# scroll-tech/zkevm-circuits

Hardware: NVIDIA H100
Metric: SuperCircuit-shaped k=20 create_proof seconds (halo2 KZG/SHPLONK, Blake2b transcript) (lower is better)
Workload: dtype u256 (8x u32 Montgomery limbs, BN254 Fr/Fq)

## Files before the change

### zkevm-circuits_b200/csrc/expr.cu

```cuda
#include <type_traits>
#include "common.cuh"
#include "expr.cuh"

namespace zkb {

struct ExprLaunch {
    const Instr *code;
    uint32_t ncode;
    const Fr *const *cols;
    const Fr *consts;
    Fr *const *outs;
    uint32_t log_n;
    uint32_t out_stride;
    uint32_t out_offset;
};

template <int NREGS, int THREADS, bool SMEM>
struct RegFile {
    uint4 *lo, *hi;
    Fr loc[SMEM ? 1 : NREGS];
    __device__ __forceinline__ RegFile(uint4 *base) : lo(base + threadIdx.x), hi(base + NREGS * THREADS + threadIdx.x) {}
    __device__ __forceinline__ Fr get(uint32_t r) const {
        if (!SMEM) return loc[r];
        const uint4 a = lo[r * THREADS], b = hi[r * THREADS];
// ... 61 lines not shown
        case OP_MUL_RC + FORM_RK: x = regs.get(in.a); y = cst(in.imm); goto mul;
        case OP_MUL_RC + FORM_KR: x = cst(in.imm); y = regs.get(in.a); goto mul;
        case OP_MUL_RC + FORM_CC: x = col(in.imm); y = col(arg()); goto mul;
        case OP_MUL_RC + FORM_CK: x = col(in.imm); y = cst(arg()); goto mul;
        case OP_MUL_RC + FORM_KC: x = cst(in.imm); y = col(arg()); goto mul;
        case OP_NEG: regs.set(in.dst, fp_neg(regs.get(in.a))); continue;
        case OP_FLAG:
            if constexpr (FLAG) {
                const uint32_t b = __ballot_sync(0xffffffffu, tid < (1u << L.log_n) && !regs.get(in.a).is_zero());
                const uint32_t word = tid >> 5;
                if ((threadIdx.x & 31) == 0 && word < L.words) L.bits[(size_t)in.imm * L.words + word] = b;
            }
            continue;
        case OP_HORNER: case OP_HORNER_C:
            if constexpr (!FLAG) acc = fp_add(fp_mul(acc, cst(in.imm)), in.op == OP_HORNER ? regs.get(in.a) : col(arg()));
            continue;
        case OP_HORNER2: case OP_HORNER2_C:
            if constexpr (!FLAG) acc2 = fp_add(fp_mul(acc2, cst(in.imm)), in.op == OP_HORNER2 ? regs.get(in.a) : col(arg()));
            continue;
        case OP_FOLD: case OP_FOLD_C:
            if constexpr (FLAG) continue;
            else { x = acc; y = cst(in.imm); z = in.op == OP_FOLD ? regs.get(in.a) : col(arg()); w = acc2; goto mac; }
        case OP_HORNER_M: case OP_HORNER2_M:
            if constexpr (FLAG) continue;
            else if constexpr (!SMEM) {
                const Fr t = fp_mul(regs.get(in.a), regs.get(in.b));
                if (in.op == OP_HORNER_M) acc = fp_add(fp_mul(acc, cst(in.imm)), t);
                else acc2 = fp_add(fp_mul(acc2, cst(in.imm)), t);
                continue;
            } else { x = in.op == OP_HORNER_M ? acc : acc2; y = cst(in.imm); z = regs.get(in.a); w = regs.get(in.b); goto mac; }
        case OP_STORE:
            if constexpr (!FLAG) fp_store(L.outs[in.imm] + (size_t)row * L.out_stride + L.out_offset, regs.get(in.a));
            continue;
        case OP_STOREACC:
            if constexpr (!FLAG) fp_store(L.outs[in.imm & 0xffu] + (size_t)row * L.out_stride + L.out_offset, fp_mul(acc, cst(in.imm >> 8)));
            continue;
        case OP_CLEARACC: acc = Fr::zero(); continue;
        default: continue;
        }
    add: regs.set(in.dst, fp_add(x, y)); continue;
    sub: regs.set(in.dst, fp_sub(x, y)); continue;
    mul: regs.set(in.dst, fp_mul(x, y)); continue;
    mac: {
        const Fr r = fp_mul_add_mul(x, y, z, w);
        if (in.op == OP_HORNER2_M) acc2 = r;
        else {
            acc = r;
            if (in.op != OP_HORNER_M) acc2 = Fr::zero();
        }
    }
    }
}

template <int NREGS, int THREADS, bool SMEM>
__global__ void __launch_bounds__(THREADS) expr_kernel(ExprLaunch L) {
    const uint32_t row = blockIdx.x * blockDim.x + threadIdx.x;
    if (row >= (1u << L.log_n)) return;
    run_program<NREGS, THREADS, SMEM>(L, row);
}

template <int NREGS, int THREADS, bool SMEM>
__global__ void __launch_bounds__(THREADS) expr_flag_kernel(FlagLaunch L) {
    run_program<NREGS, THREADS, SMEM>(L, blockIdx.x * blockDim.x + threadIdx.x);
}

template <class Launch, int NREGS, int THREADS, void (*KERNEL)(Launch)>
static int32_t launch_smem(const Launch &L, uint32_t n, cudaStream_t st) {
    constexpr size_t bytes = (size_t)NREGS * THREADS * 32;
    static bool attr_set[64] = {};
    int dev = 0;
    cudaGetDevice(&dev);
    if (bytes > 48 * 1024 && dev < 64 && !attr_set[dev]) {
        ZKB_CUDA(cudaFuncSetAttribute(KERNEL, cudaFuncAttributeMaxDynamicSharedMemorySize, (int)bytes));
        attr_set[dev] = true;
    }
    KERNEL<<<(n + THREADS - 1) / THREADS, THREADS, bytes, st>>>(L);
    return ZKB_OK;
}

int32_t expr_run_device(zkb_ctx *ctx, const Instr *d_code, uint32_t ncode, int nregs, const Fr *const *d_cols, const Fr *d_consts,
                        Fr *const *d_outs, uint32_t log_n, uint32_t out_stride, uint32_t out_offset, cudaStream_t st) {
    ExprLaunch L{d_code, ncode, d_cols, d_consts, d_outs, log_n, out_stride, out_offset};
    const uint32_t n = 1u << log_n;
    const unsigned blocks = (n + 127) / 128;
    ProfScope ps_(ctx, PROF_EXPR, st);
    if (nregs <= 8) ZKB_TRY((launch_smem<ExprLaunch, 8, 128, expr_kernel<8, 128, true>>(L, n, st)));
    else if (nregs <= 16) ZKB_TRY((launch_smem<ExprLaunch, 16, 128, expr_kernel<16, 128, true>>(L, n, st)));
    else expr_kernel<64, 128, false><<<blocks, 128, 0, st>>>(L);
    ctx->launches++;
    ZKB_CUDA(cudaGetLastError());
    return ZKB_OK;
}

int32_t expr_flag_run_device(zkb_ctx *ctx, const Instr *d_code, uint32_t ncode, int nregs, const Fr *const *d_cols, const Fr *d_consts,
                             uint32_t *bits, uint32_t words, uint32_t log_n, cudaStream_t st) {
    FlagLaunch L{d_code, ncode, d_cols, d_consts, bits, words, log_n};
    const uint32_t n = 1u << log_n;
    if (nregs <= 8) ZKB_TRY((launch_smem<FlagLaunch, 8, 128, expr_flag_kernel<8, 128, true>>(L, n, st)));
    else if (nregs <= 16) ZKB_TRY((launch_smem<FlagLaunch, 16, 128, expr_flag_kernel<16, 128, true>>(L, n, st)));
    else expr_flag_kernel<64, 128, false><<<(n + 127) / 128, 128, 0, st>>>(L);
    ctx->launches++;
    ZKB_CUDA(cudaGetLastError());
    return ZKB_OK;
}

}
```

### zkevm-circuits_b200/csrc/expr.cuh

```cuda
#pragma once
#include <stdint.h>
#include <algorithm>
#include <array>
#include <map>
#include <string>
#include <tuple>
#include <vector>
#include "common.cuh"

namespace zkb {

enum : uint8_t {
    OP_LOADCOL = 0,
    OP_LOADCONST = 1,
    OP_ADD = 2,
    OP_SUB = 3,
    OP_MUL = 4,
    OP_NEG = 5,
    OP_HORNER = 6,
    OP_STORE = 7,
    OP_STOREACC = 8,
    OP_CLEARACC = 9,
    OP_HORNER2 = 10,
    OP_FOLD = 11,
    OP_FLAG = 12,
    OP_ARG = 13,
    FORM_RC = 0, FORM_CR = 1, FORM_RK = 2, FORM_KR = 3, FORM_CC = 4, FORM_CK = 5, FORM_KC = 6,
    OP_ADD_RC = 16,
    OP_SUB_RC = 24,
    OP_MUL_RC = 32,
    OP_HORNER_C = 40,
    OP_HORNER2_C = 41,
    OP_FOLD_C = 42,
    OP_HORNER_M = 43,
    OP_HORNER2_M = 44,
};

struct alignas(8) Instr {
    uint8_t op, dst, a, b;
    uint32_t imm;
};

constexpr int EXPR_MAX_REGS = 64;

struct ENode {
    uint8_t kind;
    uint32_t a, b;
};

class ExprBuilder {
public:
    std::vector<ENode> nodes;
    std::vector<Fr> consts;
    std::vector<uint32_t> degree;

    uint32_t col(uint32_t slot, int32_t rot) { return intern(0, slot, (uint32_t)rot); }
    uint32_t constant(const Fr &v) {
        std::array<uint32_t, 8> key;
        for (int i = 0; i < 8; ++i) key[i] = v.l[i];
        auto it = const_index.find(key);
        uint32_t idx;
        if (it == const_index.end()) {
            idx = (uint32_t)consts.size();
            consts.push_back(v);
            const_index.emplace(key, idx);
        } else idx = it->second;
        return intern(1, idx, 0);
    }
    uint32_t add(uint32_t x, uint32_t y) { return intern(2, x, y); }
    uint32_t sub(uint32_t x, uint32_t y) { return intern(3, x, y); }
    uint32_t mul(uint32_t x, uint32_t y) { return intern(4, x, y); }
    uint32_t neg(uint32_t x) { return intern(5, x, 0); }
    uint32_t const_slot(const Fr &v) {
        uint32_t n = constant(v);
        return nodes[n].a;
    }
    void columns(uint32_t root, std::vector<char> &seen, std::vector<char> &used) const {
        std::vector<uint32_t> stack{root};
        while (!stack.empty()) {
            const uint32_t v = stack.back();
            stack.pop_back();
            if (seen[v]) continue;
            seen[v] = 1;
            const ENode &e = nodes[v];
            if (e.kind == 0) used[e.a] = 1;
            else if (e.kind >= 2) {
                stack.push_back(e.a);
                if (e.kind != 5) stack.push_back(e.b);
            }
        }
    }

private:
    std::map<std::tuple<uint8_t, uint32_t, uint32_t>, uint32_t> index;
    std::map<std::array<uint32_t, 8>, uint32_t> const_index;
    uint32_t intern(uint8_t kind, uint32_t a, uint32_t b) {
        auto key = std::make_tuple(kind, a, b);
        auto it = index.find(key);
        if (it != index.end()) return it->second;
        nodes.push_back(ENode{kind, a, b});
        degree.push_back(kind == 0 ? 1 : kind == 1 ? 0 : kind == 4 ? degree[a] + degree[b] : kind == 5 ? degree[a] : std::max(degree[a], degree[b]));
        index.emplace(key, (uint32_t)nodes.size() - 1);
        return (uint32_t)nodes.size() - 1;
    }
};

class ProgramBuilder {
public:
    explicit ProgramBuilder(ExprBuilder &eb) : eb(eb) {}
    std::vector<Instr> code;
    int max_regs_used = 0;
    std::string error;

    enum RootAction { HORNER, STORE, HORNER2, FOLD, FLAG };
    struct Root { uint32_t node; RootAction action; uint32_t imm; };
    bool scope(const std::vector<Root> &roots);
    void clear_acc() { code.push_back(Instr{OP_CLEARACC, 0, 0, 0, 0}); }
    void store_acc(uint32_t out_slot, uint32_t scale_const_index) {
        code.push_back(Instr{OP_STOREACC, 0, 0, 0, out_slot | (scale_const_index << 8)});
    }

private:
    ExprBuilder &eb;
    void fuse(size_t begin);
    static void merge_products(std::vector<Instr> &code);
};

inline void ProgramBuilder::fuse(size_t begin) {
    auto is_arith = [](uint8_t op) { return op == OP_ADD || op == OP_SUB || op == OP_MUL; };
    auto is_root = [](uint8_t op) { return op == OP_HORNER || op == OP_HORNER2 || op == OP_FOLD; };
    auto is_load = [](uint8_t op) { return op == OP_LOADCOL || op == OP_LOADCONST; };
    auto reads = [&](const Instr &in, int s) {
        if (is_arith(in.op)) return true;
        return s == 0 && (in.op == OP_NEG || is_root(in.op) || in.op == OP_STORE || in.op == OP_FLAG);
    };
    auto writes = [&](const Instr &in) { return is_load(in.op) || is_arith(in.op) || in.op == OP_NEG; };
    const size_t end = code.size();
    std::vector<std::array<int64_t, 2>> src(end - begin, {-1, -1});
    for (size_t i = begin; i < end; ++i) {
        if (!is_load(code[i].op)) continue;
        const uint8_t r = code[i].dst;
        int uses = 0, slot = -1;
        size_t user = 0;
        for (size_t j = i + 1; j < end && uses < 2; ++j) {
            for (int s = 0; s < 2; ++s)
                if (reads(code[j], s) && (s == 0 ? code[j].a : code[j].b) == r) { ++uses; user = j; slot = s; }
            if (writes(code[j]) && code[j].dst == r) break;
        }
        if (uses != 1) continue;
        const uint8_t op = code[user].op;
        if (is_arith(op) || (is_root(op) && code[i].op == OP_LOADCOL)) src[user - begin][slot] = (int64_t)i;
    }
    auto kind = [&](const std::array<int64_t, 2> &s, int k) { return s[k] < 0 ? 'R' : code[s[k]].op == OP_LOADCOL ? 'C' : 'K'; };
    std::vector<bool> fused(end - begin, false);
    for (auto &s : src) {
        if (kind(s, 0) == 'K' && kind(s, 1) == 'K') s[1] = -1;
        for (int k = 0; k < 2; ++k)
            if (s[k] >= 0) fused[s[k] - begin] = true;
    }
    std::vector<Instr> out;
    for (size_t i = begin; i < end; ++i) {
        const Instr in = code[i];
        const auto &s = src[i - begin];
        if (fused[i - begin]) continue;
        if (s[0] < 0 && s[1] < 0) { out.push_back(in); continue; }
        if (is_root(in.op)) {
            const uint8_t op = in.op == OP_HORNER ? OP_HORNER_C : in.op == OP_HORNER2 ? OP_HORNER2_C : OP_FOLD_C;
            out.push_back(Instr{op, 0, 0, 0, in.imm});
            out.push_back(Instr{OP_ARG, 0, 0, 0, code[s[0]].imm});
            continue;
        }
        const char ka = kind(s, 0), kb = kind(s, 1);
        const int form = ka == 'R' ? (kb == 'C' ? FORM_RC : FORM_RK)
                       : kb == 'R' ? (ka == 'C' ? FORM_CR : FORM_KR)
                       : ka == 'C' ? (kb == 'C' ? FORM_CC : FORM_CK) : FORM_KC;
        const uint8_t base = in.op == OP_ADD ? OP_ADD_RC : in.op == OP_SUB ? OP_SUB_RC : OP_MUL_RC;
        const int first = s[0] >= 0 ? 0 : 1;
        const uint8_t reg = ka == 'R' ? in.a : in.b;
        out.push_back(Instr{(uint8_t)(base + form), in.dst, (uint8_t)(form < FORM_CC ? reg : 0), 0, code[s[first]].imm});
// ... 4 lines not shown
    code.insert(code.end(), out.begin(), out.end());
}

inline void ProgramBuilder::merge_products(std::vector<Instr> &code) {
    const size_t n = code.size();
    auto reg_reads = [](const Instr &in, int s) {
        const uint8_t op = in.op;
        if (op == OP_ADD || op == OP_SUB || op == OP_MUL) return true;
        if (s != 0) return false;
        if (op == OP_NEG || op == OP_HORNER || op == OP_HORNER2 || op == OP_FOLD || op == OP_STORE || op == OP_FLAG) return true;
        return op >= OP_ADD_RC && op < OP_MUL_RC + 8 && (op & 7) < FORM_CC;
    };
    auto reg_writes = [](const Instr &in) {
        const uint8_t op = in.op;
        return op == OP_LOADCOL || op == OP_LOADCONST || op == OP_ADD || op == OP_SUB || op == OP_MUL || op == OP_NEG ||
               (op >= OP_ADD_RC && op < OP_MUL_RC + 8);
    };
    std::vector<int64_t> reader(n, -1);
    for (size_t i = 0; i < n; ++i) {
        const Instr &m = code[i];
        if (m.op != OP_MUL) continue;
        int uses = 0;
        size_t user = 0;
        for (size_t j = i + 1; j < n && uses < 2; ++j) {
            for (int s = 0; s < 2; ++s)
                if (reg_reads(code[j], s) && (s == 0 ? code[j].a : code[j].b) == m.dst) { ++uses; user = j; }
            if (reg_writes(code[j]) && code[j].dst == m.dst) break;
        }
        if (uses != 1) continue;
        bool intact = true;
        for (size_t j = i + 1; j < user; ++j)
            if (reg_writes(code[j]) && (code[j].dst == m.a || code[j].dst == m.b)) intact = false;
        if (intact) reader[i] = (int64_t)user;
    }
    std::vector<int64_t> prod(n, -1);
    for (size_t i = 0; i < n; ++i)
        if (reader[i] >= 0 && (code[reader[i]].op == OP_HORNER || code[reader[i]].op == OP_HORNER2)) prod[reader[i]] = (int64_t)i;
    std::vector<bool> merged(n, false);
    std::vector<Instr> out;
    for (size_t j = 0; j < n; ++j) {
        Instr in = code[j];
        if (prod[j] >= 0) {
            in = Instr{(uint8_t)(in.op == OP_HORNER ? OP_HORNER_M : OP_HORNER2_M), 0, code[prod[j]].a, code[prod[j]].b, in.imm};
            merged[prod[j]] = true;
        }
        out.push_back(in);
    }
    code.clear();
    for (size_t j = 0; j < n; ++j)
        if (!merged[j]) code.push_back(out[j]);
}

inline bool ProgramBuilder::scope(const std::vector<Root> &roots) {
    const size_t begin = code.size();
    std::map<uint32_t, int> refs;
    std::vector<uint32_t> stack;
    std::map<uint32_t, bool> seen;
    for (auto &r : roots) {
        refs[r.node]++;
        if (!seen[r.node]) { seen[r.node] = true; stack.push_back(r.node); }
    }
    while (!stack.empty()) {
        uint32_t n = stack.back();
        stack.pop_back();
        const ENode &e = eb.nodes[n];
        if (e.kind >= 2) {
            uint32_t ch[2] = {e.a, e.b};
            int nch = e.kind == 5 ? 1 : 2;
            for (int i = 0; i < nch; ++i) {
                refs[ch[i]]++;
                if (!seen[ch[i]]) { seen[ch[i]] = true; stack.push_back(ch[i]); }
            }
        }
    }
    std::map<uint32_t, int> reg_of;
    std::vector<int> free_regs;
    for (int i = EXPR_MAX_REGS - 1; i >= 0; --i) free_regs.push_back(i);
    auto alloc = [&]() -> int {
        if (free_regs.empty()) return -1;
        int r = free_regs.back();
        free_regs.pop_back();
        if (r + 1 > max_regs_used) max_regs_used = r + 1;
        return r;
    };
    auto release_use = [&](uint32_t n) {
        if (--refs[n] == 0) {
            free_regs.push_back(reg_of[n]);
            reg_of.erase(n);
        }
    };
    struct Frame { uint32_t node; int state; };
    for (auto &r : roots) {
        if (!reg_of.count(r.node)) {
            std::vector<Frame> st;
            st.push_back({r.node, 0});
            while (!st.empty()) {
                Frame &f = st.back();
                const ENode e = eb.nodes[f.node];
                if (reg_of.count(f.node)) { st.pop_back(); continue; }
                if (e.kind < 2) {
                    int rg = alloc();
                    if (rg < 0) { error = "expression needs more than 64 live registers"; return false; }
                    if (e.kind == 0) code.push_back(Instr{OP_LOADCOL, (uint8_t)rg, 0, 0, (e.a & 0xffffu) | ((uint32_t)(uint16_t)(int16_t)(int32_t)e.b << 16)});
                    else code.push_back(Instr{OP_LOADCONST, (uint8_t)rg, 0, 0, e.a});
                    reg_of[f.node] = rg;
                    st.pop_back();
                    continue;
                }
                const int nch = e.kind == 5 ? 1 : 2;
                if (f.state == 0) {
                    f.state = 1;
                    if (!reg_of.count(e.a)) { st.push_back({e.a, 0}); continue; }
                }
                if (f.state == 1) {
                    f.state = 2;
                    if (nch == 2 && !reg_of.count(e.b)) { st.push_back({e.b, 0}); continue; }
                }
                const int ra = reg_of[e.a];
                const int rb = nch == 2 ? reg_of[e.b] : 0;
                const uint32_t me = f.node;
                release_use(e.a);
                if (nch == 2) release_use(e.b);
                int rg = alloc();
                if (rg < 0) { error = "expression needs more than 64 live registers"; return false; }
                uint8_t op = e.kind == 2 ? OP_ADD : e.kind == 3 ? OP_SUB : e.kind == 4 ? OP_MUL : OP_NEG;
                code.push_back(Instr{op, (uint8_t)rg, (uint8_t)ra, (uint8_t)rb, 0});
                reg_of[me] = rg;
                st.pop_back();
            }
        }
        const int rr = reg_of[r.node];
        if (r.action == HORNER) code.push_back(Instr{OP_HORNER, 0, (uint8_t)rr, 0, r.imm});
        else if (r.action == HORNER2) code.push_back(Instr{OP_HORNER2, 0, (uint8_t)rr, 0, r.imm});
        else if (r.action == FOLD) code.push_back(Instr{OP_FOLD, 0, (uint8_t)rr, 0, r.imm});
        else if (r.action == FLAG) code.push_back(Instr{OP_FLAG, 0, (uint8_t)rr, 0, r.imm});
        else code.push_back(Instr{OP_STORE, 0, (uint8_t)rr, 0, r.imm});
        release_use(r.node);
    }
    fuse(begin);
    return true;
}

int32_t expr_run_device(zkb_ctx *ctx, const Instr *d_code, uint32_t ncode, int nregs, const Fr *const *d_cols, const Fr *d_consts,
                        Fr *const *d_outs, uint32_t log_n, uint32_t out_stride, uint32_t out_offset, cudaStream_t st);
int32_t expr_flag_run_device(zkb_ctx *ctx, const Instr *d_code, uint32_t ncode, int nregs, const Fr *const *d_cols, const Fr *d_consts,
                             uint32_t *bits, uint32_t words, uint32_t log_n, cudaStream_t st);

struct DeviceProgram {
    Instr *code = nullptr;
    uint32_t ncode = 0;
    int nregs = 0;
    Fr *consts = nullptr;
};
inline int32_t upload_program(DevPool &pool, const ProgramBuilder &pb, const ExprBuilder &eb, DeviceProgram &dp, cudaStream_t st) {
    dp.ncode = (uint32_t)pb.code.size();
    dp.nregs = pb.max_regs_used;
    ZKB_TRY(pool.alloc(pb.code.size() * sizeof(Instr) + 8, (void **)&dp.code));
    ZKB_TRY(pool.alloc(eb.consts.size() * sizeof(Fr) + 32, (void **)&dp.consts));
    ZKB_CUDA(cudaMemcpyAsync(dp.code, pb.code.data(), pb.code.size() * sizeof(Instr), cudaMemcpyHostToDevice, st));
    ZKB_CUDA(cudaMemcpyAsync(dp.consts, eb.consts.data(), eb.consts.size() * sizeof(Fr), cudaMemcpyHostToDevice, st));
    ZKB_CUDA(cudaStreamSynchronize(st));
    return ZKB_OK;
}
template <class T>
inline int32_t upload_table(DevPool &pool, const std::vector<T *> &host, T ***dev, cudaStream_t st) {
    ZKB_TRY(pool.alloc(host.size() * sizeof(T *) + 8, (void **)dev));
    ZKB_CUDA(cudaMemcpyAsync(*dev, host.data(), host.size() * sizeof(T *), cudaMemcpyHostToDevice, st));
    ZKB_CUDA(cudaStreamSynchronize(st));
    return ZKB_OK;
// ... 16 lines not shown
```

### zkevm-circuits_b200/csrc/prover.cu

```cuda
#include "common.cuh"
#include "csf.cuh"
#include "expr.cuh"
#include "lookup.cuh"
#include "transcript.cuh"
#include <algorithm>
#include <memory>
#include <string.h>
#include <stdlib.h>
#include <time.h>

namespace zkb {

__global__ void set_one_kernel(Fr *a, uint64_t idx) { fp_store(a + idx, Fr::one()); }
__global__ void fill_range_one_kernel(Fr *a, uint64_t from, uint64_t to) {
    uint64_t i = from + blockIdx.x * (uint64_t)blockDim.x + threadIdx.x;
    if (i < to) fp_store(a + i, Fr::one());
}
__global__ void mul_arrays_kernel(const Fr *__restrict__ a, const Fr *__restrict__ b, Fr *__restrict__ out, uint64_t n) {
    uint64_t i = blockIdx.x * (uint64_t)blockDim.x + threadIdx.x;
    if (i < n) fp_store(out + i, fp_mul(fp_load(a + i), fp_load(b + i)));
}
__global__ void scale_const_kernel(Fr *__restrict__ a, Fr c, uint64_t n) {
    uint64_t i = blockIdx.x * (uint64_t)blockDim.x + threadIdx.x;
    if (i < n) fp_store(a + i, fp_mul(fp_load(a + i), c));
// ... 784 lines not shown
        const uint32_t g = group_of(eb.degree[sel] + d);
        const int64_t s = next, r = (int64_t)rests.size();
        for (uint32_t v : rests)
            if (!emit(g, {{v, ProgramBuilder::HORNER2, eb.const_slot(y)}})) return false;
        const uint32_t fold = eb.const_slot(fp_pow_u64(y, (uint64_t)(last[g] < 0 ? r : s - last[g] - 1 + r)));
        if (!emit(g, {{sel, ProgramBuilder::FOLD, fold}})) return false;
        reads[g].push_back(sel);
        reads[g].insert(reads[g].end(), rests.begin(), rests.end());
        last[g] = s + r - 1;
        next += r;
        count[g] += (uint32_t)r;
        return true;
    }
    Fr tail(uint32_t g) const { return fp_pow_u64(y, (uint64_t)(next - 1 - last[g])); }
};

static int32_t quotient_gates(const Csf &cs, const std::vector<Fr> &challenges, QuotientGroups &qg, const SlotMap &sm,
                              std::vector<int64_t> &memo) {
    ExprBuilder &qeb = qg.eb;
    auto selector_split = [&](uint32_t gnode, uint32_t &sel, uint32_t &rest) -> bool {
        const auto &nd = cs.nodes[gnode];
        if (nd[0] != N_MUL) return false;
        for (int side = 0; side < 2; ++side) {
            const uint32_t a = nd[1 + side], b = nd[2 - side];
            if (cs.nodes[a][0] == N_FIXED) { sel = a; rest = b; return true; }
        }
        return false;
    };
    auto same_query = [&](uint32_t a, uint32_t b) { return cs.nodes[a][1] == cs.nodes[b][1] && cs.nodes[a][2] == cs.nodes[b][2]; };
    for (size_t gi = 0; gi < cs.gates.size();) {
        uint32_t sel = 0, rest = 0;
        size_t run = 1;
        if (selector_split(cs.gates[gi], sel, rest)) {
            uint32_t s2 = 0, r2 = 0;
            while (gi + run < cs.gates.size() && run < 4096 && selector_split(cs.gates[gi + run], s2, r2) && same_query(sel, s2)) ++run;
        }
        if (run < 2) {
            if (!qg.scope({translate(cs, cs.gates[gi], qeb, sm, challenges, memo)})) { set_error("gate: %s", qg.error.c_str()); return ZKB_ERR_ARG; }
            ++gi;
            continue;
        }
        std::vector<uint32_t> rests(run);
        for (size_t t = 0; t < run; ++t) {
            uint32_t s2 = 0, r2 = 0;
            selector_split(cs.gates[gi + t], s2, r2);
            rests[t] = translate(cs, r2, qeb, sm, challenges, memo);
        }
        if (!qg.run(rests, translate(cs, sel, qeb, sm, challenges, memo))) { set_error("gate: %s", qg.error.c_str()); return ZKB_ERR_ARG; }
        gi += run;
    }
    return ZKB_OK;
}

static int32_t evaluate_h(zkb_session *s, ProofState &ps, StageTrace &trace) {
    zkb_pk *pk = s->pk;
    zkb_ctx *ctx = pk->ctx;
    const Csf &cs = pk->cs;
    const uint64_t n = pk->n;
    const uint32_t k = cs.k;
    const Fr one = Fr::one();
    cudaStream_t st = ctx->stream;
    DevPool &pool = s->pool;
    const SlotMap &sm = pk->sm;
    std::vector<Fr *> qpolys = pk_quotient_polys(pk);
    put_columns(qpolys, sm.advice0, ps.adv_polys);
    put_columns(qpolys, sm.instance0, s->inst_polys);
    put_columns(qpolys, sm.z0, ps.z_polys);
    put_columns(qpolys, sm.phi0, ps.phi_polys);
    put_columns(qpolys, sm.m0, ps.m_polys);
    ZKB_ARG(qpolys.size() < 65536);

    const uint32_t E = pk->E;
    uint32_t G = 1;
    while ((1u << (G - 1)) < E) ++G;
    ExprBuilder qeb;
    std::vector<ProgramBuilder> qpbs(G, ProgramBuilder(qeb));
    std::vector<ProgramBuilder *> qpb_ptrs;
    for (auto &p : qpbs) qpb_ptrs.push_back(&p);
    QuotientGroups qg(qeb, ps.y, E, qpb_ptrs);
    std::vector<int64_t> memo(cs.nodes.size(), -1);
    ZKB_TRY(quotient_gates(cs, s->challenges, qg, sm, memo));
    auto lactive = [&]() { return qeb.sub(qeb.sub(qeb.constant(one), qeb.col(sm.l_last, 0)), qeb.col(sm.l_blind, 0)); };
    if (pk->nsets) {
        const uint32_t z0 = qeb.col(sm.z0, 0), zl = qeb.col(sm.z0 + pk->nsets - 1, 0);
        if (!qg.scope({qeb.mul(qeb.sub(qeb.constant(one), z0), qeb.col(sm.l0, 0))})) return ZKB_ERR_ARG;
        if (!qg.scope({qeb.mul(qeb.sub(qeb.mul(zl, zl), zl), qeb.col(sm.l_last, 0))})) return ZKB_ERR_ARG;
        for (uint32_t i = 1; i < pk->nsets; ++i) {
            const uint32_t t = qeb.mul(qeb.sub(qeb.col(sm.z0 + i, 0), qeb.col(sm.z0 + i - 1, -(int32_t)(cs.bf + 1))), qeb.col(sm.l0, 0));
            if (!qg.scope({t})) return ZKB_ERR_ARG;
        }
        for (uint32_t si = 0; si < pk->nsets; ++si) {
            uint32_t left = qeb.col(sm.z0 + si, 1), right = qeb.col(sm.z0 + si, 0);
            perm_set_products(cs, sm, pk->chunk, si, ps.beta, ps.gamma, qeb, right, left);
            if (!qg.scope({qeb.mul(qeb.sub(left, right), lactive())})) { set_error("permutation: %s", qg.error.c_str()); return ZKB_ERR_ARG; }
        }
    }
    for (size_t l = 0; l < cs.lookups.size(); ++l) {
        const CsfLookup &lk = cs.lookups[l];
        std::vector<uint32_t> fsb;
        for (auto &inp : lk.inputs) fsb.push_back(qeb.add(compress_exprs(cs, inp, qeb, sm, s->challenges, memo, ps.theta), qeb.constant(ps.beta)));
        const uint32_t tb = qeb.add(compress_exprs(cs, lk.table, qeb, sm, s->challenges, memo, ps.theta), qeb.constant(ps.beta));
        uint32_t prod = fsb[0];
        for (size_t j = 1; j < fsb.size(); ++j) prod = qeb.mul(prod, fsb[j]);
        uint32_t ssum = 0;
        bool have_sum = false;
        for (size_t i = 0; i < fsb.size(); ++i) {
            uint32_t pr = 0;
            bool have = false;
            for (size_t j = 0; j < fsb.size(); ++j) {
                if (j == i) continue;
                pr = have ? qeb.mul(pr, fsb[j]) : fsb[j];
                have = true;
            }
            if (!have) pr = qeb.constant(one);
            ssum = have_sum ? qeb.add(ssum, pr) : pr;
            have_sum = true;
        }
        const uint32_t phi = qeb.col(sm.phi0 + (uint32_t)l, 0), phi_next = qeb.col(sm.phi0 + (uint32_t)l, 1), m = qeb.col(sm.m0 + (uint32_t)l, 0);
        const uint32_t lhs = qeb.mul(qeb.mul(tb, prod), qeb.sub(phi_next, phi));
        const uint32_t rhs = qeb.sub(qeb.mul(tb, ssum), qeb.mul(m, prod));
        if (!qg.scope({qeb.mul(phi, qeb.col(sm.l0, 0)), qeb.mul(phi, qeb.col(sm.l_last, 0)), qeb.mul(qeb.sub(lhs, rhs), lactive())})) {
            set_error("lookup %zu: %s", l, qg.error.c_str());
            return ZKB_ERR_ARG;
        }
    }
    auto on_part = [&](uint32_t g, uint32_t j) { return j % (E >> g) == 0; };
    std::vector<uint32_t> groups;
    for (uint32_t g = 0; g < G; ++g)
        if (qg.count[g]) groups.push_back(g);
    std::vector<std::vector<uint32_t>> scale_idx(G, std::vector<uint32_t>(E, 0));
    for (uint32_t g : groups) {
        const Fr tail = qg.tail(g);
        for (uint32_t j = 0; j < E; ++j)
            if (on_part(g, j)) scale_idx[g][j] = qeb.const_slot(fp_mul(pk->t_inv[j], tail));
    }
    std::vector<DeviceProgram> qdp(G);
    std::vector<size_t> base_len(G, 0);
    for (uint32_t g : groups) {
        base_len[g] = qpbs[g].code.size();
        qpbs[g].store_acc(0, scale_idx[g][0]);
        ZKB_TRY(upload_program(pool, qpbs[g], qeb, qdp[g], st));
    }
    auto cached = [&](size_t i) { return !pk->coset_cache.empty() && pk->coset_cache[0][i]; };
    std::vector<int> reader(qpolys.size(), -1);
    {
        std::vector<char> seen(qeb.nodes.size());
        for (uint32_t g : groups) {
            std::fill(seen.begin(), seen.end(), 0);
            std::vector<char> used(qpolys.size(), 0);
            for (uint32_t v : qg.reads[g]) qeb.columns(v, seen, used);
            for (size_t i = 0; i < used.size(); ++i)
                if (used[i]) reader[i] = (int)g;
        }
    }
    if (trace.on) {
        for (uint32_t g : groups) {
            size_t instrs = 0, ntts = 0;
            for (const Instr &in : qpbs[g].code) instrs += in.op != OP_ARG;
            for (size_t i = 0; i < qpolys.size(); ++i) ntts += !cached(i) && reader[i] == (int)g;
            fprintf(stderr, "[zkb trace] quotient group m = %-2u %6u constraints %7zu instructions/row %5zu coset NTTs\n", 1u << g, qg.count[g],
                    instrs, ntts << g);
        }
    }
    trace.mark("quotient program build+upload");

    Fr *slab, *pows;
    ZKB_TRY(pool.fr(qpolys.size() * n, &slab));
    ZKB_TRY(pool.fr(n, &pows));
    ZKB_TRY(pool.fr(pk->N, &ps.h_ext));
    ps.h_group.assign(G, nullptr);
    for (uint32_t g : groups) {
        if (g + 1 == G) ps.h_group[g] = ps.h_ext;
        else ZKB_TRY(pool.fr(n << g, &ps.h_group[g]));
    }
    std::vector<Fr *> qcols(qpolys.size());
    for (size_t i = 0; i < qpolys.size(); ++i) qcols[i] = slab + i * n;
    const Deal dq(ctx, E);
    std::vector<std::vector<uint32_t>> row_of(G, std::vector<uint32_t>(E, 0));
    size_t blk_rows = 0;
    Fr *rows_slab = nullptr;
    if (dq.on) {
        std::vector<size_t> next_row(dq.P, 0);
        for (uint32_t j = 0; j < E; ++j)
            for (uint32_t g : groups) next_row[j / dq.blk] += on_part(g, j);
        blk_rows = *std::max_element(next_row.begin(), next_row.end());
        for (int r = 0; r < dq.P; ++r) next_row[r] = (size_t)r * blk_rows;
        for (uint32_t j = 0; j < E; ++j)
            for (uint32_t g : groups)
                if (on_part(g, j)) row_of[g][j] = (uint32_t)next_row[j / dq.blk]++;
        ZKB_TRY(pool.fr((size_t)dq.P * blk_rows * n, &rows_slab));
    }
    std::vector<Fr **> d_hout(G, nullptr);
    for (uint32_t g : groups) ZKB_TRY(upload_table(pool, std::vector<Fr *>{dq.on ? rows_slab : ps.h_group[g]}, &d_hout[g], st));
    Fr **d_qcols = nullptr;
    ZKB_TRY(pool.alloc(qcols.size() * sizeof(Fr *) + 8, (void **)&d_qcols));
    for (uint32_t j = 0; j < E; ++j) {
        if (!dq.mine(j)) continue;
        std::vector<Fr *> ntt_src, ntt_dst;
        for (size_t i = 0; i < qpolys.size(); ++i)
            if (!cached(i) && reader[i] >= 0 && on_part((uint32_t)reader[i], j)) { ntt_src.push_back(qpolys[i]); ntt_dst.push_back(qcols[i]); }
        if (!ntt_src.empty()) {
            ZKB_TRY(fr_powers_device(ctx, pk->coset_gen(j), n, pows, st));
            ZKB_TRY(ntt_many(pk, ntt_src, ntt_dst, pk->omega, nullptr, pows, st));
        }
        std::vector<Fr *> cols_j = qcols;
        for (size_t i = 0; i < qpolys.size(); ++i)
            if (cached(i)) cols_j[i] = pk->coset_cache[j][i];
        ZKB_CUDA(cudaMemcpyAsync(d_qcols, cols_j.data(), cols_j.size() * sizeof(Fr *), cudaMemcpyHostToDevice, st));
        std::vector<Instr> tails(G);
        for (uint32_t g : groups) {
            if (!on_part(g, j)) continue;
            tails[g] = Instr{OP_STOREACC, 0, 0, 0, 0u | (scale_idx[g][j] << 8)};
            ZKB_CUDA(cudaMemcpyAsync(qdp[g].code + base_len[g], &tails[g], sizeof(Instr), cudaMemcpyHostToDevice, st));
            const DeviceProgram &dp = qdp[g];
            if (dq.on) ZKB_TRY(expr_run_device(ctx, dp.code, dp.ncode, dp.nregs, d_qcols, dp.consts, d_hout[g], k, 1, (uint32_t)(row_of[g][j] * n), st));
            else ZKB_TRY(expr_run_device(ctx, dp.code, dp.ncode, dp.nregs, d_qcols, dp.consts, d_hout[g], k, 1u << g, j / (E >> g), st));
        }
        ZKB_CUDA(cudaStreamSynchronize(st));
    }
    if (dq.on) {
        ZKB_TRY(comm_allgather(ctx, rows_slab + (size_t)dq.rank * blk_rows * n, rows_slab, blk_rows * n * sizeof(Fr), st));
        std::vector<std::vector<uint32_t>> rows(G);
        for (uint32_t g : groups) {
            for (uint32_t jj = 0; jj < (1u << g); ++jj) rows[g].push_back(row_of[g][jj * (E >> g)]);
            uint32_t *d_rows = nullptr;
            ZKB_TRY(pool.alloc(rows[g].size() * sizeof(uint32_t), (void **)&d_rows));
            ZKB_CUDA(cudaMemcpyAsync(d_rows, rows[g].data(), rows[g].size() * sizeof(uint32_t), cudaMemcpyHostToDevice, st));
            interleave_rows_kernel<<<(unsigned)(((n << g) + 255) / 256), 256, 0, st>>>(rows_slab, d_rows, ps.h_group[g], k, 1u << g);
            ctx->launches++;
// ... 279 lines not shown
    ZKB_TRY(shplonk(s, ps));
    trace.mark("shplonk");
    ZKB_TRY(s->tr.status());
    s->finished = true;
    return ZKB_OK;
}

}

extern "C" int32_t zkb_prove_finish(zkb_session *s, const uint64_t *z_blinds, const uint64_t *phi_blinds, const uint64_t *random_poly,
                                    uint8_t *proof_out, uint64_t proof_cap, uint64_t *proof_len) {
    ZKB_ARG(s && proof_len);
    zkb_pk *pk = s->pk;
    if (!s->finished) {
        ZKB_ARG(random_poly != nullptr);
        if (s->next_phase != pk->cs.nphases) { set_error("zkb_prove_finish: advice phases incomplete"); return ZKB_ERR_STATE; }
        ZKB_ARG((pk->nsets == 0 || z_blinds) && (pk->cs.lookups.empty() || phi_blinds));
        ZKB_CUDA(cudaSetDevice(pk->ctx->device));
        ZKB_TRY(prove_finish_stages(s, z_blinds, phi_blinds, random_poly));
    }
    const std::vector<uint8_t> &proof = s->tr.proof();
    *proof_len = proof.size();
    if (proof_out) {
        if (proof_cap < proof.size()) { set_error("zkb_prove_finish: buffer of %llu bytes, proof has %llu (kept in the session: call again)",
                                             (unsigned long long)proof_cap, (unsigned long long)proof.size()); return ZKB_ERR_ARG; }
        memcpy(proof_out, proof.data(), proof.size());
    }
    return ZKB_OK;
}

static int32_t gate_program(const Csf &cs, const SlotMap &sm, int32_t mode, const uint64_t *challenges, const uint64_t y[4], const uint64_t scale[4],
                            ExprBuilder &eb, ProgramBuilder &pb) {
    ZKB_ARG(cs.nch == 0 || challenges);
    const std::vector<Fr> ch = host_challenges(challenges, cs.nch);
    std::vector<int64_t> memo(cs.nodes.size(), -1);
    if (mode == 0) {
        std::vector<ProgramBuilder::Root> roots;
        for (size_t i = 0; i < cs.gates.size(); ++i) roots.push_back({translate(cs, cs.gates[i], eb, sm, ch, memo), ProgramBuilder::STORE, (uint32_t)i});
        if (!pb.scope(roots)) { set_error("gates: %s", pb.error.c_str()); return ZKB_ERR_ARG; }
        return ZKB_OK;
    }
    Fr yv, sv;
    memcpy(yv.l, y, sizeof(Fr));
    memcpy(sv.l, scale, sizeof(Fr));
    QuotientGroups qg(eb, yv, 1, {&pb});
    ZKB_TRY(quotient_gates(cs, ch, qg, sm, memo));
    pb.store_acc(0, eb.const_slot(sv));
    return ZKB_OK;
}

extern "C" int32_t zkb_expr_eval_dev(zkb_ctx *ctx, const uint32_t *csf, uint64_t csf_words, int32_t mode, const uint64_t *challenges,
                                     const uint64_t y[4], const uint64_t scale[4], const uint64_t *const *columns_dev,
                                     uint64_t *const *outs_dev, uint32_t out_stride, uint32_t out_offset, uint32_t *nregs_out, void *stream) {
    ZKB_ARG(ctx && csf && columns_dev && outs_dev && (mode == 0 || mode == 1));
    ZKB_ARG(mode == 0 ? out_stride == 1 && out_offset == 0 : y && scale && out_stride >= 1);
    ZKB_CUDA(cudaSetDevice(ctx->device));
    Csf cs;
    ZKB_TRY(load_csf(csf, csf_words, cs));
    const SlotMap sm(cs, 0);
    ExprBuilder eb;
    ProgramBuilder pb(eb);
    ZKB_TRY(gate_program(cs, sm, mode, challenges, y, scale, eb, pb));
    cudaStream_t st = pick_stream(ctx, stream);
    const std::vector<Fr *> cols((Fr *const *)columns_dev, (Fr *const *)columns_dev + sm.sigma0);
    std::vector<Fr *> outs(mode == 0 ? cs.gates.size() : 1);
    for (size_t i = 0; i < outs.size(); ++i) outs[i] = (Fr *)outs_dev[i];
    DevPool pool;
    pool.ctx = ctx;
    Fr **d_cols = nullptr, **d_outs = nullptr;
    DeviceProgram dp;
    ZKB_TRY(upload_table(pool, cols, &d_cols, st));
    ZKB_TRY(upload_table(pool, outs, &d_outs, st));
    ZKB_TRY(upload_program(pool, pb, eb, dp, st));
    ZKB_TRY(expr_run_device(ctx, dp.code, dp.ncode, dp.nregs, d_cols, dp.consts, d_outs, cs.k, out_stride, out_offset, st));
    ZKB_CUDA(cudaStreamSynchronize(st));
    if (nregs_out) *nregs_out = (uint32_t)dp.nregs;
    return ZKB_OK;
}

extern "C" int32_t zkb_expr_program(const uint32_t *csf, uint64_t csf_words, int32_t mode, const uint64_t *challenges, const uint64_t y[4],
                                    const uint64_t scale[4], uint64_t *code_out, uint64_t cap, uint64_t *ncode_out, uint32_t *nregs_out) {
    ZKB_ARG(csf && ncode_out && (mode == 0 || mode == 1) && (mode == 0 || (y && scale)) && (code_out || cap == 0));
    Csf cs;
    ZKB_TRY(load_csf(csf, csf_words, cs));
    ExprBuilder eb;
    ProgramBuilder pb(eb);
    ZKB_TRY(gate_program(cs, SlotMap(cs, 0), mode, challenges, y, scale, eb, pb));
    static_assert(sizeof(Instr) == sizeof(uint64_t), "one program word per instruction");
    *ncode_out = pb.code.size();
    if (nregs_out) *nregs_out = (uint32_t)pb.max_regs_used;
    if (cap) memcpy(code_out, pb.code.data(), std::min<uint64_t>(cap, pb.code.size()) * sizeof(Instr));
    return ZKB_OK;
}
```

Before: 1.570.

## Schedule quotient expression programs to minimize live registers and add smaller smem variants

Adds an optional scheduling mode to the expression program builder. It emits each scope twice, once in the existing order and once in a Sethi-Ullman order, linear-scan compacts the register assignment of both, and keeps whichever needs fewer registers. The quotient-group builders enable this mode, and new 7- and 12-register shared-memory kernel variants are added (the 7-register one with a min-blocks launch bound), so fewer registers mean smaller per-block shared memory and higher occupancy. The cost is extra host-side program build time from emitting twice plus the recursive need computation, and the min-blocks bound can force register spills.

```diff
diff --git a/zkevm-circuits_b200/csrc/expr.cu b/zkevm-circuits_b200/csrc/expr.cu
--- a/zkevm-circuits_b200/csrc/expr.cu
+++ b/zkevm-circuits_b200/csrc/expr.cu
@@ -137,15 +137,15 @@
     }
 }
 
-template <int NREGS, int THREADS, bool SMEM>
-__global__ void __launch_bounds__(THREADS) expr_kernel(ExprLaunch L) {
+template <int NREGS, int THREADS, bool SMEM, int MINB = 0>
+__global__ void __launch_bounds__(THREADS, MINB) expr_kernel(ExprLaunch L) {
     const uint32_t row = blockIdx.x * blockDim.x + threadIdx.x;
     if (row >= (1u << L.log_n)) return;
     run_program<NREGS, THREADS, SMEM>(L, row);
 }
 
-template <int NREGS, int THREADS, bool SMEM>
-__global__ void __launch_bounds__(THREADS) expr_flag_kernel(FlagLaunch L) {
+template <int NREGS, int THREADS, bool SMEM, int MINB = 0>
+__global__ void __launch_bounds__(THREADS, MINB) expr_flag_kernel(FlagLaunch L) {
     run_program<NREGS, THREADS, SMEM>(L, blockIdx.x * blockDim.x + threadIdx.x);
 }
 
@@ -169,7 +169,9 @@
     const uint32_t n = 1u << log_n;
     const unsigned blocks = (n + 127) / 128;
     ProfScope ps_(ctx, PROF_EXPR, st);
-    if (nregs <= 8) ZKB_TRY((launch_smem<ExprLaunch, 8, 128, expr_kernel<8, 128, true>>(L, n, st)));
+    if (nregs <= 7) ZKB_TRY((launch_smem<ExprLaunch, 7, 128, expr_kernel<7, 128, true, 7>>(L, n, st)));
+    else if (nregs <= 8) ZKB_TRY((launch_smem<ExprLaunch, 8, 128, expr_kernel<8, 128, true>>(L, n, st)));
+    else if (nregs <= 12) ZKB_TRY((launch_smem<ExprLaunch, 12, 128, expr_kernel<12, 128, true>>(L, n, st)));
     else if (nregs <= 16) ZKB_TRY((launch_smem<ExprLaunch, 16, 128, expr_kernel<16, 128, true>>(L, n, st)));
     else expr_kernel<64, 128, false><<<blocks, 128, 0, st>>>(L);
     ctx->launches++;
@@ -181,7 +183,9 @@
                              uint32_t *bits, uint32_t words, uint32_t log_n, cudaStream_t st) {
     FlagLaunch L{d_code, ncode, d_cols, d_consts, bits, words, log_n};
     const uint32_t n = 1u << log_n;
-    if (nregs <= 8) ZKB_TRY((launch_smem<FlagLaunch, 8, 128, expr_flag_kernel<8, 128, true>>(L, n, st)));
+    if (nregs <= 7) ZKB_TRY((launch_smem<FlagLaunch, 7, 128, expr_flag_kernel<7, 128, true, 7>>(L, n, st)));
+    else if (nregs <= 8) ZKB_TRY((launch_smem<FlagLaunch, 8, 128, expr_flag_kernel<8, 128, true>>(L, n, st)));
+    else if (nregs <= 12) ZKB_TRY((launch_smem<FlagLaunch, 12, 128, expr_flag_kernel<12, 128, true>>(L, n, st)));
     else if (nregs <= 16) ZKB_TRY((launch_smem<FlagLaunch, 16, 128, expr_flag_kernel<16, 128, true>>(L, n, st)));
     else expr_flag_kernel<64, 128, false><<<(n + 127) / 128, 128, 0, st>>>(L);
     ctx->launches++;
diff --git a/zkevm-circuits_b200/csrc/expr.cuh b/zkevm-circuits_b200/csrc/expr.cuh
--- a/zkevm-circuits_b200/csrc/expr.cuh
+++ b/zkevm-circuits_b200/csrc/expr.cuh
@@ -2,6 +2,7 @@
 #include <stdint.h>
 #include <algorithm>
 #include <array>
+#include <functional>
 #include <map>
 #include <string>
 #include <tuple>
@@ -107,7 +108,7 @@
 
 class ProgramBuilder {
 public:
-    explicit ProgramBuilder(ExprBuilder &eb) : eb(eb) {}
+    explicit ProgramBuilder(ExprBuilder &eb, bool schedule = false) : eb(eb), schedule(schedule) {}
     std::vector<Instr> code;
     int max_regs_used = 0;
     std::string error;
@@ -122,9 +123,76 @@
 
 private:
     ExprBuilder &eb;
+    bool schedule;
+    bool emit_scope(const std::vector<Root> &roots, bool sethi_ullman);
     void fuse(size_t begin);
     static void merge_products(std::vector<Instr> &code);
-};
+    bool compact(size_t begin, int &peak);
+};
+
+inline bool instr_reads(const Instr &in, int s) {
+    const uint8_t op = in.op;
+    if (op == OP_ADD || op == OP_SUB || op == OP_MUL || op == OP_HORNER_M || op == OP_HORNER2_M) return true;
+    if (s != 0) return false;
+    if (op == OP_NEG || op == OP_HORNER || op == OP_HORNER2 || op == OP_FOLD || op == OP_STORE || op == OP_FLAG) return true;
+    return op >= OP_ADD_RC && op < OP_MUL_RC + 8 && (op & 7) < FORM_CC;
+}
+inline bool instr_writes(const Instr &in) {
+    const uint8_t op = in.op;
+    return op == OP_LOADCOL || op == OP_LOADCONST || op == OP_ADD || op == OP_SUB || op == OP_MUL || op == OP_NEG ||
+           (op >= OP_ADD_RC && op < OP_MUL_RC + 8);
+}
+
+inline bool ProgramBuilder::compact(size_t begin, int &peak) {
+    const size_t end = code.size();
+    std::vector<std::array<bool, 2>> last(end - begin, {false, false});
+    std::vector<bool> unread(end - begin, false);
+    std::vector<int64_t> pending(256, -1);
+    std::vector<int64_t> writer(256, -1);
+    auto close = [&](int reg) {
+        if (pending[reg] >= 0) last[pending[reg] / 2][pending[reg] % 2] = true;
+        else if (writer[reg] >= 0) unread[writer[reg]] = true;
+    };
+    for (size_t i = begin; i < end; ++i) {
+        const Instr &in = code[i];
+        if (in.op == OP_ARG) continue;
+        for (int s = 0; s < 2; ++s)
+            if (instr_reads(in, s)) pending[s ? in.b : in.a] = (int64_t)(i - begin) * 2 + s;
+        if (instr_writes(in)) {
+            close(in.dst);
+            pending[in.dst] = -1;
+            writer[in.dst] = (int64_t)(i - begin);
+        }
+    }
+    for (int r = 0; r < 256; ++r) close(r);
+    std::vector<int> now(256, -1);
+    std::vector<bool> busy(EXPR_MAX_REGS, false);
+    peak = 0;
+    for (size_t i = begin; i < end; ++i) {
+        Instr &in = code[i];
+        if (in.op == OP_ARG) continue;
+        const uint8_t old_a = in.a, old_b = in.b;
+        int freed[2] = {-1, -1};
+        for (int s = 0; s < 2; ++s) {
+            if (!instr_reads(in, s)) continue;
+            const uint8_t old = s ? old_b : old_a;
+            const int r = now[old];
+            if (s) in.b = (uint8_t)r; else in.a = (uint8_t)r;
+            if (last[i - begin][s]) freed[s] = r;
+        }
+        for (int s = 0; s < 2; ++s)
+            if (freed[s] >= 0) busy[freed[s]] = false;
+        if (!instr_writes(in)) continue;
+        int r = 0;
+        while (r < EXPR_MAX_REGS && busy[r]) ++r;
+        if (r == EXPR_MAX_REGS) { error = "expression needs more than 64 live registers"; return false; }
+        busy[r] = !unread[i - begin];
+        peak = std::max(peak, r + 1);
+        now[in.dst] = r;
+        in.dst = (uint8_t)r;
+    }
+    return true;
+}
 
 inline void ProgramBuilder::fuse(size_t begin) {
     auto is_arith = [](uint8_t op) { return op == OP_ADD || op == OP_SUB || op == OP_MUL; };
@@ -235,6 +303,23 @@
 }
 
 inline bool ProgramBuilder::scope(const std::vector<Root> &roots) {
+    if (!schedule) return emit_scope(roots, false);
+    const size_t begin = code.size();
+    int peak_su = 0, peak_w = 0;
+    const bool ok_su = emit_scope(roots, true) && compact(begin, peak_su);
+    const std::vector<Instr> su(code.begin() + begin, code.end());
+    code.resize(begin);
+    const bool ok_w = emit_scope(roots, false) && compact(begin, peak_w);
+    if (!ok_su && !ok_w) return false;
+    if (!ok_w || (ok_su && peak_su < peak_w)) {
+        code.resize(begin);
+        code.insert(code.end(), su.begin(), su.end());
+    }
+    max_regs_used = std::max(max_regs_used, !ok_w ? peak_su : !ok_su ? peak_w : std::min(peak_su, peak_w));
+    return true;
+}
+
+inline bool ProgramBuilder::emit_scope(const std::vector<Root> &roots, bool sethi_ullman) {
     const size_t begin = code.size();
     std::map<uint32_t, int> refs;
     std::vector<uint32_t> stack;
@@ -258,13 +343,34 @@
     }
     std::map<uint32_t, int> reg_of;
     std::vector<int> free_regs;
-    for (int i = EXPR_MAX_REGS - 1; i >= 0; --i) free_regs.push_back(i);
+    for (int i = (schedule ? 256 : EXPR_MAX_REGS) - 1; i >= 0; --i) free_regs.push_back(i);
     auto alloc = [&]() -> int {
         if (free_regs.empty()) return -1;
         int r = free_regs.back();
         free_regs.pop_back();
-        if (r + 1 > max_regs_used) max_regs_used = r + 1;
+        if (!schedule && r + 1 > max_regs_used) max_regs_used = r + 1;
         return r;
+    };
+    const std::map<uint32_t, int> uses = refs;
+    std::map<uint32_t, int> need_memo;
+    auto held = [&](uint32_t v) { return reg_of.count(v) || eb.nodes[v].kind >= 2 || uses.at(v) > 1 ? 1 : 0; };
+    std::function<int(uint32_t)> need = [&](uint32_t v) -> int {
+        if (reg_of.count(v)) return 0;
+        const ENode &e = eb.nodes[v];
+        if (e.kind < 2) return uses.at(v) > 1 ? 1 : 0;
+        auto it = need_memo.find(v);
+        if (it != need_memo.end()) return it->second;
+        int r = std::max(need(e.a), 1);
+        if (e.kind != 5) {
+            const int na = need(e.a), nb = need(e.b);
+            r = std::max(1, std::min(std::max(na, held(e.a) + nb), std::max(nb, held(e.b) + na)));
+        }
+        return need_memo[v] = r;
+    };
+    auto b_first = [&](const ENode &e) {
+        if (!sethi_ullman || e.kind == 5) return false;
+        const int na = need(e.a), nb = need(e.b);
+        return std::max(nb, held(e.b) + na) < std::max(na, held(e.a) + nb);
     };
     auto release_use = [&](uint32_t n) {
         if (--refs[n] == 0) {
@@ -292,12 +398,15 @@
                 }
                 const int nch = e.kind == 5 ? 1 : 2;
                 if (f.state == 0) {
-                    f.state = 1;
-                    if (!reg_of.count(e.a)) { st.push_back({e.a, 0}); continue; }
+                    need_memo.clear();
+                    f.state = b_first(e) ? 3 : 1;
+                    const uint32_t first = f.state == 3 ? e.b : e.a;
+                    if (!reg_of.count(first)) { st.push_back({first, 0}); continue; }
                 }
-                if (f.state == 1) {
+                if (f.state == 1 || f.state == 3) {
+                    const uint32_t second = f.state == 3 ? e.a : e.b;
                     f.state = 2;
-                    if (nch == 2 && !reg_of.count(e.b)) { st.push_back({e.b, 0}); continue; }
+                    if (nch == 2 && !reg_of.count(second)) { st.push_back({second, 0}); continue; }
                 }
                 const int ra = reg_of[e.a];
                 const int rb = nch == 2 ? reg_of[e.b] : 0;
diff --git a/zkevm-circuits_b200/csrc/prover.cu b/zkevm-circuits_b200/csrc/prover.cu
--- a/zkevm-circuits_b200/csrc/prover.cu
+++ b/zkevm-circuits_b200/csrc/prover.cu
@@ -882,7 +882,7 @@
     uint32_t G = 1;
     while ((1u << (G - 1)) < E) ++G;
     ExprBuilder qeb;
-    std::vector<ProgramBuilder> qpbs(G, ProgramBuilder(qeb));
+    std::vector<ProgramBuilder> qpbs(G, ProgramBuilder(qeb, true));
     std::vector<ProgramBuilder *> qpb_ptrs;
     for (auto &p : qpbs) qpb_ptrs.push_back(&p);
     QuotientGroups qg(qeb, ps.y, E, qpb_ptrs);
@@ -966,8 +966,8 @@
             size_t instrs = 0, ntts = 0;
             for (const Instr &in : qpbs[g].code) instrs += in.op != OP_ARG;
             for (size_t i = 0; i < qpolys.size(); ++i) ntts += !cached(i) && reader[i] == (int)g;
-            fprintf(stderr, "[zkb trace] quotient group m = %-2u %6u constraints %7zu instructions/row %5zu coset NTTs\n", 1u << g, qg.count[g],
-                    instrs, ntts << g);
+            fprintf(stderr, "[zkb trace] quotient group m = %-2u %6u constraints %7zu instructions/row %5zu coset NTTs %3d registers\n", 1u << g,
+                    qg.count[g], instrs, ntts << g, qpbs[g].max_regs_used);
         }
     }
     trace.mark("quotient program build+upload");
@@ -1368,14 +1368,14 @@
 extern "C" int32_t zkb_expr_eval_dev(zkb_ctx *ctx, const uint32_t *csf, uint64_t csf_words, int32_t mode, const uint64_t *challenges,
                                      const uint64_t y[4], const uint64_t scale[4], const uint64_t *const *columns_dev,
                                      uint64_t *const *outs_dev, uint32_t out_stride, uint32_t out_offset, uint32_t *nregs_out, void *stream) {
-    ZKB_ARG(ctx && csf && columns_dev && outs_dev && (mode == 0 || mode == 1));
+    ZKB_ARG(ctx && csf && columns_dev && outs_dev && mode >= 0 && mode <= 2);
     ZKB_ARG(mode == 0 ? out_stride == 1 && out_offset == 0 : y && scale && out_stride >= 1);
     ZKB_CUDA(cudaSetDevice(ctx->device));
     Csf cs;
     ZKB_TRY(load_csf(csf, csf_words, cs));
     const SlotMap sm(cs, 0);
     ExprBuilder eb;
-    ProgramBuilder pb(eb);
+    ProgramBuilder pb(eb, mode == 2);
     ZKB_TRY(gate_program(cs, sm, mode, challenges, y, scale, eb, pb));
     cudaStream_t st = pick_stream(ctx, stream);
     const std::vector<Fr *> cols((Fr *const *)columns_dev, (Fr *const *)columns_dev + sm.sigma0);
@@ -1396,11 +1396,11 @@
 
 extern "C" int32_t zkb_expr_program(const uint32_t *csf, uint64_t csf_words, int32_t mode, const uint64_t *challenges, const uint64_t y[4],
                                     const uint64_t scale[4], uint64_t *code_out, uint64_t cap, uint64_t *ncode_out, uint32_t *nregs_out) {
-    ZKB_ARG(csf && ncode_out && (mode == 0 || mode == 1) && (mode == 0 || (y && scale)) && (code_out || cap == 0));
+    ZKB_ARG(csf && ncode_out && mode >= 0 && mode <= 2 && (mode == 0 || (y && scale)) && (code_out || cap == 0));
     Csf cs;
     ZKB_TRY(load_csf(csf, csf_words, cs));
     ExprBuilder eb;
-    ProgramBuilder pb(eb);
+    ProgramBuilder pb(eb, mode == 2);
     ZKB_TRY(gate_program(cs, SlotMap(cs, 0), mode, challenges, y, scale, eb, pb));
     static_assert(sizeof(Instr) == sizeof(uint64_t), "one program word per instruction");
     *ncode_out = pb.code.size();
```

Result: faster. 1.542 (median of 6 runs) (-1.8%).

## Precombine lookup input advice columns into theta-compressed polys before coset NTTs

Applied to the files above, without the earlier changes.

Finds lookup input sets made only of plain advice columns (optionally sharing one cofactor and rotation) whose columns are read nowhere else. For each such set it builds one theta-weighted linear combination polynomial up front, so the quotient evaluates a single coset NTT of that combination rather than one per advice column. The coset slab is now sized only for columns that are actually transformed. This trades extra lincomb work and memory for fewer coset NTTs and fewer per-row instructions, and it depends on the 'elsewhere' analysis being correct.

```diff
diff --git a/zkevm-circuits_b200/csrc/prover.cu b/zkevm-circuits_b200/csrc/prover.cu
--- a/zkevm-circuits_b200/csrc/prover.cu
+++ b/zkevm-circuits_b200/csrc/prover.cu
@@ -860,6 +860,91 @@
     return ZKB_OK;
 }
 
+struct InputCombos {
+    struct Set { int32_t combo = -1; uint32_t cofactor = NO_NODE; int32_t rot = 0; };
+    std::vector<std::vector<Set>> sets;
+    std::vector<std::vector<uint32_t>> columns;
+};
+static InputCombos lookup_input_combos(const Csf &cs, ExprBuilder &qeb, const SlotMap &sm, const std::vector<Fr> &challenges,
+                                       std::vector<int64_t> &memo) {
+    std::vector<char> reads_cells(cs.nodes.size(), 0);
+    for (size_t i = 0; i < cs.nodes.size(); ++i) {
+        const auto &nd = cs.nodes[i];
+        reads_cells[i] = nd[0] == N_ADVICE || nd[0] == N_INSTANCE || (nd[0] >= N_NEG && reads_cells[nd[1]]) ||
+                         ((nd[0] == N_ADD || nd[0] == N_MUL) && reads_cells[nd[2]]);
+    }
+    std::vector<char> elsewhere(cs.na, 0), seen(cs.nodes.size(), 0);
+    auto read_by = [&](uint32_t root) {
+        std::vector<uint32_t> stack{root};
+        while (!stack.empty()) {
+            const uint32_t v = stack.back();
+            stack.pop_back();
+            if (seen[v]) continue;
+            seen[v] = 1;
+            const auto &nd = cs.nodes[v];
+            if (nd[0] == N_ADVICE) elsewhere[nd[1]] = 1;
+            if (nd[0] >= N_NEG) stack.push_back(nd[1]);
+            if (nd[0] == N_ADD || nd[0] == N_MUL) stack.push_back(nd[2]);
+        }
+    };
+    for (uint32_t g : cs.gates) read_by(g);
+    for (auto &pc : cs.perm)
+        if (pc[0] == N_ADVICE) elsewhere[pc[1]] = 1;
+    InputCombos out;
+    std::vector<std::vector<std::vector<uint32_t>>> cols(cs.lookups.size());
+    out.sets.resize(cs.lookups.size());
+    for (size_t l = 0; l < cs.lookups.size(); ++l) {
+        const CsfLookup &lk = cs.lookups[l];
+        for (uint32_t v : lk.table) read_by(v);
+        out.sets[l].resize(lk.inputs.size());
+        cols[l].resize(lk.inputs.size());
+        for (size_t i = 0; i < lk.inputs.size(); ++i) {
+            const std::vector<uint32_t> &inp = lk.inputs[i];
+            InputCombos::Set &set = out.sets[l][i];
+            bool ok = inp.size() >= 2;
+            for (size_t c = 0; c < inp.size() && ok; ++c) {
+                const auto &nd = cs.nodes[inp[c]];
+                uint32_t adv = inp[c], cof = NO_NODE;
+                if (nd[0] == N_MUL) {
+                    const int side = cs.nodes[nd[1]][0] == N_ADVICE && !reads_cells[nd[2]] ? 0 : 1;
+                    adv = nd[1 + side];
+                    cof = nd[2 - side];
+                    if (reads_cells[cof]) ok = false;
+                }
+                if (!ok || cs.nodes[adv][0] != N_ADVICE) { ok = false; break; }
+                const uint32_t s = cof == NO_NODE ? NO_NODE : translate(cs, cof, qeb, sm, challenges, memo);
+                const int32_t rot = (int32_t)cs.nodes[adv][2];
+                if (c == 0) { set.cofactor = s; set.rot = rot; }
+                else ok = s == set.cofactor && rot == set.rot;
+                cols[l][i].push_back(cs.nodes[adv][1]);
+            }
+            if (ok) set.combo = 0;
+            else for (uint32_t v : inp) read_by(v);
+        }
+    }
+    for (bool changed = true; changed;) {
+        changed = false;
+        for (size_t l = 0; l < cs.lookups.size(); ++l)
+            for (size_t i = 0; i < cols[l].size(); ++i) {
+                InputCombos::Set &set = out.sets[l][i];
+                if (set.combo < 0 || std::none_of(cols[l][i].begin(), cols[l][i].end(), [&](uint32_t c) { return elsewhere[c]; })) continue;
+                set.combo = -1;
+                for (uint32_t c : cols[l][i]) elsewhere[c] = 1;
+                changed = true;
+            }
+    }
+    std::map<std::vector<uint32_t>, int32_t> index;
+    for (size_t l = 0; l < cs.lookups.size(); ++l)
+        for (size_t i = 0; i < cols[l].size(); ++i) {
+            InputCombos::Set &set = out.sets[l][i];
+            if (set.combo < 0) continue;
+            auto it = index.emplace(cols[l][i], (int32_t)out.columns.size()).first;
+            if (it->second == (int32_t)out.columns.size()) out.columns.push_back(cols[l][i]);
+            set.combo = it->second;
+        }
+    return out;
+}
+
 static int32_t evaluate_h(zkb_session *s, ProofState &ps, StageTrace &trace) {
     zkb_pk *pk = s->pk;
     zkb_ctx *ctx = pk->ctx;
@@ -876,7 +961,6 @@
     put_columns(qpolys, sm.z0, ps.z_polys);
     put_columns(qpolys, sm.phi0, ps.phi_polys);
     put_columns(qpolys, sm.m0, ps.m_polys);
-    ZKB_ARG(qpolys.size() < 65536);
 
     const uint32_t E = pk->E;
     uint32_t G = 1;
@@ -903,10 +987,20 @@
             if (!qg.scope({qeb.mul(qeb.sub(left, right), lactive())})) { set_error("permutation: %s", qg.error.c_str()); return ZKB_ERR_ARG; }
         }
     }
+    const InputCombos combos = lookup_input_combos(cs, qeb, sm, s->challenges, memo);
     for (size_t l = 0; l < cs.lookups.size(); ++l) {
         const CsfLookup &lk = cs.lookups[l];
         std::vector<uint32_t> fsb;
-        for (auto &inp : lk.inputs) fsb.push_back(qeb.add(compress_exprs(cs, inp, qeb, sm, s->challenges, memo, ps.theta), qeb.constant(ps.beta)));
+        for (size_t i = 0; i < lk.inputs.size(); ++i) {
+            const InputCombos::Set &set = combos.sets[l][i];
+            uint32_t f;
+            if (set.combo < 0) f = compress_exprs(cs, lk.inputs[i], qeb, sm, s->challenges, memo, ps.theta);
+            else {
+                f = qeb.col(sm.slots + (uint32_t)set.combo, set.rot);
+                if (set.cofactor != NO_NODE) f = qeb.mul(set.cofactor, f);
+            }
+            fsb.push_back(qeb.add(f, qeb.constant(ps.beta)));
+        }
         const uint32_t tb = qeb.add(compress_exprs(cs, lk.table, qeb, sm, s->challenges, memo, ps.theta), qeb.constant(ps.beta));
         uint32_t prod = fsb[0];
         for (size_t j = 1; j < fsb.size(); ++j) prod = qeb.mul(prod, fsb[j]);
@@ -932,6 +1026,23 @@
             return ZKB_ERR_ARG;
         }
     }
+    std::vector<std::vector<Fr>> coefs(combos.columns.size());
+    Fr *combo_polys = nullptr;
+    if (!combos.columns.empty()) ZKB_TRY(pool.fr(combos.columns.size() * n, &combo_polys));
+    for (size_t c = 0; c < combos.columns.size(); ++c) {
+        const std::vector<uint32_t> &cols = combos.columns[c];
+        std::vector<Fr *> polys(cols.size());
+        coefs[c].resize(cols.size());
+        Fr p = one;
+        for (size_t t = cols.size(); t-- > 0;) {
+            polys[t] = ps.adv_polys[cols[t]];
+            coefs[c][t] = p;
+            p = fp_mul(p, ps.theta);
+        }
+        ZKB_TRY(lincomb(pk, pool, polys, coefs[c], combo_polys + c * n, false, st));
+        qpolys.push_back(combo_polys + c * n);
+    }
+    ZKB_ARG(qpolys.size() < 65536);
     auto on_part = [&](uint32_t g, uint32_t j) { return j % (E >> g) == 0; };
     std::vector<uint32_t> groups;
     for (uint32_t g = 0; g < G; ++g)
@@ -949,7 +1060,7 @@
         qpbs[g].store_acc(0, scale_idx[g][0]);
         ZKB_TRY(upload_program(pool, qpbs[g], qeb, qdp[g], st));
     }
-    auto cached = [&](size_t i) { return !pk->coset_cache.empty() && pk->coset_cache[0][i]; };
+    auto cached = [&](size_t i) { return !pk->coset_cache.empty() && i < pk->coset_cache[0].size() && pk->coset_cache[0][i]; };
     std::vector<int> reader(qpolys.size(), -1);
     {
         std::vector<char> seen(qeb.nodes.size());
@@ -972,8 +1083,13 @@
     }
     trace.mark("quotient program build+upload");
 
+    std::vector<Fr *> qcols(qpolys.size(), nullptr);
+    size_t transformed = 0;
+    for (size_t i = 0; i < qpolys.size(); ++i) transformed += !cached(i) && reader[i] >= 0;
     Fr *slab, *pows;
-    ZKB_TRY(pool.fr(qpolys.size() * n, &slab));
+    ZKB_TRY(pool.fr(transformed * n, &slab));
+    for (size_t i = 0, t = 0; i < qpolys.size(); ++i)
+        if (!cached(i) && reader[i] >= 0) qcols[i] = slab + t++ * n;
     ZKB_TRY(pool.fr(n, &pows));
     ZKB_TRY(pool.fr(pk->N, &ps.h_ext));
     ps.h_group.assign(G, nullptr);
@@ -981,8 +1097,6 @@
         if (g + 1 == G) ps.h_group[g] = ps.h_ext;
         else ZKB_TRY(pool.fr(n << g, &ps.h_group[g]));
     }
-    std::vector<Fr *> qcols(qpolys.size());
-    for (size_t i = 0; i < qpolys.size(); ++i) qcols[i] = slab + i * n;
     const Deal dq(ctx, E);
     std::vector<std::vector<uint32_t>> row_of(G, std::vector<uint32_t>(E, 0));
     size_t blk_rows = 0;
```

Result: faster. 1.570 before, 1.510 after, median of 6 (-3.8%).
